# freewym/espresso

Measured on AMD Instinct MI355X. Metric: audio-hours/sec training (LibriSpeech Conformer-12 + CTC), higher is better.
Workload: dtype bf16; 1 GPU; LibriSpeech 960h Conformer-12 + CTC update step, <=26000 frames & <=24 utts per GPU, V=5004, on-GPU fbank+CMVN+SpecAugment, dropout 0.1, clip 2.0, Adam; parallelism=dp1

## Files before the change

### espresso_amd/csrc/optim.hip

```cpp
#include "common.h"
#include "espresso_amd.h"

namespace {

__global__ __launch_bounds__(256) void sumsq_kernel(const float* __restrict__ g, long n, float* __restrict__ out) {
  __shared__ float sm[16];
  float s = 0.f;
  const long stride = (long)gridDim.x * blockDim.x * 4;
  for (long i = ((long)blockIdx.x * blockDim.x + threadIdx.x) * 4; i < n; i += stride) {
    if (i + 4 <= n) {
      const float4 v = *reinterpret_cast<const float4*>(g + i);
      s += v.x * v.x + v.y * v.y + v.z * v.z + v.w * v.w;
    } else {
      for (long j = i; j < n; ++j) s += g[j] * g[j];
    }
  }
  s = block_sum(s, sm);
  if (threadIdx.x == 0) atomicAdd(out, s);
}

__global__ void clip_coef_kernel(const float* __restrict__ sumsq, float pre_scale, const float* __restrict__ denom,
                                 float max_norm, float* __restrict__ coef) {
  if (denom) pre_scale = pre_scale / denom[0];
  const float norm = sqrtf(sumsq[0]) * pre_scale;
  float c = 1.f;
  if (max_norm > 0.f) c = fminf(1.f, max_norm / (norm + 1e-6f));
  if (!(fabsf(norm) < INFINITY)) c = norm;
  coef[0] = pre_scale * c;
  coef[1] = norm;
}

__global__ __launch_bounds__(256) void adam_kernel(float* __restrict__ p, float* __restrict__ g, float* __restrict__ m,
                                                   float* __restrict__ v, bf16_t* __restrict__ p_bf16, long n,
                                                   const float* __restrict__ coef, float lr, float beta1, float beta2,
                                                   float eps, float weight_decay, float step_size, int zero_grad) {
  const float gs = coef ? coef[0] : 1.f;
  const bool skip = !(gs == gs) || fabsf(gs) == INFINITY;
  const long stride = (long)gridDim.x * blockDim.x * 4;
  for (long i = ((long)blockIdx.x * blockDim.x + threadIdx.x) * 4; i < n; i += stride) {
    const int cnt = (int)((n - i) < 4 ? (n - i) : 4);
    float pv[4], gv[4], mv[4], vv[4];
    if (cnt == 4) {
      const f32x4_t a = __builtin_nontemporal_load(reinterpret_cast<const f32x4_t*>(p + i));
      const f32x4_t b = __builtin_nontemporal_load(reinterpret_cast<const f32x4_t*>(g + i));
      const f32x4_t c = __builtin_nontemporal_load(reinterpret_cast<const f32x4_t*>(m + i));
      const f32x4_t d = __builtin_nontemporal_load(reinterpret_cast<const f32x4_t*>(v + i));
      pv[0] = a.x; pv[1] = a.y; pv[2] = a.z; pv[3] = a.w;
// ... 24 lines not shown
      if (zero_grad) __builtin_nontemporal_store((f32x4_t){0.f, 0.f, 0.f, 0.f}, reinterpret_cast<f32x4_t*>(g + i));
      if (p_bf16) *reinterpret_cast<uint2*>(p_bf16 + i) = make_uint2(pack_bf2(pv[0], pv[1]), pack_bf2(pv[2], pv[3]));
    } else {
      for (int e = 0; e < cnt; ++e) {
        p[i + e] = pv[e]; m[i + e] = mv[e]; v[i + e] = vv[e];
        if (zero_grad) g[i + e] = 0.f;
        if (p_bf16) p_bf16[i + e] = f2bf(pv[e]);
      }
    }
  }
}

}

extern "C" int ea_grad_sumsq(const float* g, long n, float* out , hipStream_t stream) {
  if (n <= 0) return 0;
  long blocks = (n + 1023) / 1024;
  if (blocks > 2048) blocks = 2048;
  hipLaunchKernelGGL(sumsq_kernel, dim3((unsigned)blocks), dim3(256), 0, stream, g, n, out);
  return EA_CHECK_LAUNCH();
}
extern "C" int ea_clip_coef(const float* sumsq, float pre_scale, const float* denom_dev, float max_norm,
                            float* coef , hipStream_t stream) {
  hipLaunchKernelGGL(clip_coef_kernel, dim3(1), dim3(1), 0, stream, sumsq, pre_scale, denom_dev, max_norm, coef);
  return EA_CHECK_LAUNCH();
}
extern "C" int ea_adam_step(float* p, float* g, float* m, float* v, void* p_bf16, long n, const float* coef,
                            float lr, float beta1, float beta2, float eps, float weight_decay, int step,
                            int zero_grad, hipStream_t stream) {
  if (n <= 0) return 0;
  const double bc1 = 1.0 - pow((double)beta1, (double)step);
  const double bc2 = 1.0 - pow((double)beta2, (double)step);
  const float step_size = (float)((double)lr * sqrt(bc2) / bc1);
  long blocks = (n + 1023) / 1024;
  if (blocks > 4096) blocks = 4096;
  hipLaunchKernelGGL(adam_kernel, dim3((unsigned)blocks), dim3(256), 0, stream, p, g, m, v, (bf16_t*)p_bf16, n, coef, lr,
                     beta1, beta2, eps, weight_decay, step_size, zero_grad);
  return EA_CHECK_LAUNCH();
}
```

### espresso_amd/functional.py

```python
import collections

import ctypes
import os

import torch

from . import kernels as K

_seed_state = {"base": 0x5EED, "counter": 0}


def set_dropout_seed(seed: int):
    _seed_state["base"] = int(seed) & 0xFFFFFFFF
    _seed_state["counter"] = 0


_seed_trace = None


class trace_dropout_seeds:

    def __enter__(self):
        global _seed_trace
        self.prev, self.entries = _seed_trace, []
# ... 644 lines not shown


_CONV1_FUSED_BWD = True


def set_conv1_fused_backward(on: bool) -> bool:
    global _CONV1_FUSED_BWD
    old, _CONV1_FUSED_BWD = _CONV1_FUSED_BWD, bool(on)
    return old


def set_conv_implicit_gemm(on: bool):
    global _CONV_IGEMM
    _CONV_IGEMM = bool(on)


def _conv_igemm_ok(cin, cout, sy, sx):
    return _CONV_IGEMM and cin in (64, 128) and cout in (64, 128) and sy in (1, 2) and sx in (1, 2)


class _ConvSubsample(torch.autograd.Function):

    @staticmethod
    def forward(ctx, X, row_zero, strides, bufs, p_drop, training, bn_eps, bn_momentum, *params):
        B, T, F = X.shape
        L = len(params) // 4
        saved = []
        cfgs = []
        A = None
        Tc, Fc, Cc = T, F, 1
        for i in range(L):
            w, b, g, beta = params[4 * i: 4 * i + 4]
            rm, rv = bufs[2 * i], bufs[2 * i + 1]
            sy, sx = strides[i]
            Co = w.shape[0]
            To, Fo = (Tc - 1) // sy + 1, (Fc - 1) // sx + 1
            stats = _pool_zeros((2 * Co,), torch.float64, X.device) if training else None
            if i == 0:
                assert w.shape[1] == 1 and tuple(w.shape[2:]) == (3, 3)
                Zi = K.conv1_fwd(X, w.detach().reshape(Co, 9).contiguous(), b, B, Tc, Fc, Co, sy, sx, stats)
                col, w16 = None, None
            elif _conv_igemm_ok(Cc, Co, sy, sx):
                w16 = K.cast_f32_to_bf16(w.detach().permute(0, 2, 3, 1).reshape(Co, 9 * Cc).contiguous())
                Zi = K.conv3x3_fwd(A, w16, b, B, Tc, Fc, Cc, Co, sy, sx, stats=stats)
                col = A
            else:
                col = K.im2col3x3(A, B, Tc, Fc, Cc, sy, sx)
                w16 = K.cast_f32_to_bf16(w.detach().permute(0, 2, 3, 1).reshape(Co, 9 * Cc).contiguous())
                Zi = _new((B * To * Fo, Co), torch.bfloat16, X)
                K.gemm(col, w16, Zi, B * To * Fo, Co, 9 * Cc, lda=9 * Cc, ldb=9 * Cc, ldc=Co, bias=b)
                if training:
                    K.colstats(Zi, stats)
            n = B * To * Fo
            mr = K.bn_finalize(stats, Co, n, bn_eps, bn_momentum, rm, rv) if training else K.bn_from_running(rm, rv, bn_eps)
            A = K.bn_act_fwd(Zi, mr, g, beta, "relu")
            saved += [Zi, mr, col, w16, g, beta]
            cfgs.append((Tc, Fc, Cc, To, Fo, Co, sy, sx))
            Tc, Fc, Cc = To, Fo, Co
        out = A.view(B * Tc, Fc * Cc)
        seed = _next_seed("subsample.out", p_drop) if (training and p_drop > 0) else 0
        if seed:
            out = K.scale_dropout(out, a=1.0, drop_p=p_drop, drop_seed=seed)
        if row_zero is not None:
            K.zero_rows(out, row_zero)
        ctx.save_for_backward(X, row_zero, *[t for t in saved if t is not None])
        ctx.layout = [[t is not None for t in saved[6 * i: 6 * i + 6]] for i in range(L)]
        ctx.cfg = (B, cfgs, p_drop, seed, training, [tuple(p.shape) for p in params[0::4]])
        ctx.igemm = [i > 0 and _conv_igemm_ok(cfgs[i][2], cfgs[i][5], cfgs[i][6], cfgs[i][7]) for i in range(L)]
        ctx.weights = [params[4 * i] for i in range(L)]
        ctx.params = list(params)
        return out

    @staticmethod
    def backward(ctx, dout):
        X, row_zero, *flat = ctx.saved_tensors
        B, cfgs, p_drop, seed, training, wshapes = ctx.cfg
        L = len(cfgs)
        it = iter(flat)
# ... 59 lines not shown
                    grads[4 * i] = dWp.view(Co, 3, 3, Cc).permute(0, 3, 1, 2)
                if not training:
                    db = g.detach() * mr[1] * dbeta
                elif _grad_sink(pb, Co) is not None:
                    db = None
                wd16 = K.cast_f32_to_bf16(ctx.weights[i].detach().permute(1, 2, 3, 0).reshape(Cc, 9 * Co).contiguous())
                dA = K.conv3x3_dgrad(dZ, wd16, B, Tc, Fc, Cc, Co, sy, sx)
            else:
                dWp = torch.empty((Co, 9 * Cc), dtype=torch.float32, device=X.device)
                side.wait_stream(cur)
                with torch.cuda.stream(side):
                    _wgrad(dZ, col, n, Co, 9 * Cc, out=dWp)
                    K.colsum(dZ, db, n, Co, Co)
                grads[4 * i] = dWp.view(Co, 3, 3, Cc).permute(0, 3, 1, 2)
                dcol = _new((n, 9 * Cc), torch.bfloat16, X)
                K.gemm(dZ, w16, dcol, n, 9 * Cc, Co, lda=Co, ldb=9 * Cc, ldc=9 * Cc, b_kstrided=True)
                dA = K.col2im3x3(dcol, B, Tc, Fc, Cc, sy, sx)
            grads[4 * i + 1] = db
            if sg is None:
                grads[4 * i + 2] = dg
                grads[4 * i + 3] = dbeta
        cur.wait_stream(side)
        del keep
        return (None,) * 8 + tuple(grads)


def conv_subsample(X, row_zero, strides, params, bufs, p_drop=0.0, training=True, bn_eps=1e-5, bn_momentum=0.1):
    return _ConvSubsample.apply(X, row_zero, tuple(strides), list(bufs), p_drop, training, bn_eps, bn_momentum, *params)


_grad_ready_callback = None


def set_grad_ready_callback(fn):
    global _grad_ready_callback
    _grad_ready_callback = fn


def _ptr(t):
    return None if t is None else t.data_ptr()


class _LayerBinding:

    def __init__(self, m, kind="conformer"):
        import ctypes

        from ._lib import EaConformerLayer

        self.keep = []
        self.kind = kind
# ... 1277 lines not shown
```

### espresso_amd/kernels.py

```python
import ctypes
from typing import Optional

import torch

from . import _lib
from ._lib import EaGemmParams, check

ACT_NONE, ACT_RELU, ACT_SILU = 0, 1, 2
_ACT = {None: 0, "none": 0, "relu": 1, "silu": 2, "swish": 2}


def _stream():
    return ctypes.c_void_p(torch._C._cuda_getCurrentRawStream(torch._C._cuda_getDevice()))


def _p(t: Optional[torch.Tensor]):
    if t is None:
        return None
    if not t.is_cuda:
        raise RuntimeError("espresso_amd kernels need device tensors (no CPU path)")
    return ctypes.c_void_p(t.data_ptr())


def drop_params(p: float):
# ... 457 lines not shown
        "ea_specaugment",
    )
    return feat


def grad_sumsq(g, out):
    check(_lib.lib().ea_grad_sumsq(_p(g), g.numel(), _p(out), _stream()), "ea_grad_sumsq")
    return out


def clip_coef(sumsq, pre_scale, max_norm, coef, denom_dev=None):
    check(_lib.lib().ea_clip_coef(_p(sumsq), pre_scale, _p(denom_dev), max_norm, _p(coef), _stream()), "ea_clip_coef")
    return coef


def adam_step(p, g, m, v, p_bf16, coef, lr, beta1, beta2, eps, weight_decay, step, zero_grad=True):
    check(
        _lib.lib().ea_adam_step(_p(p), _p(g), _p(m), _p(v), _p(p_bf16), p.numel(), _p(coef), lr, beta1, beta2, eps,
                                weight_decay, step, int(zero_grad), _stream()),
        "ea_adam_step",
    )


def ctc_greedy_decode(x, in_len, B, T, V, blank, pad, ld=None, want_align=True):
    dev = x.device
    ld = x.stride(0) if ld is None else ld
    best = torch.empty(B * T, dtype=torch.int32, device=dev)
    bestv = torch.empty(B * T, dtype=torch.float32, device=dev)
    tokens = torch.empty(B, T, dtype=torch.int32, device=dev)
    align = torch.zeros(B, T, dtype=torch.int32, device=dev) if want_align else None
    out_len = torch.empty(B, dtype=torch.int32, device=dev)
    score = torch.empty(B, dtype=torch.float32, device=dev)
    check(
        _lib.lib().ea_ctc_greedy_decode(_p(x), ld, int(x.dtype == torch.bfloat16), _p(in_len), _p(best), _p(bestv), _p(tokens),
                                        _p(align), _p(out_len), _p(score), B, T, V, blank, pad, _stream()),
        "ea_ctc_greedy_decode",
    )
    return tokens, out_len, score, align


def _finish_outputs(n, nbest, max_u, device):
    return (torch.empty(n, nbest, max_u, dtype=torch.int32, device=device), torch.empty(n, nbest, dtype=torch.int32, device=device),
            torch.empty(n, nbest, dtype=torch.float32, device=device), torch.empty(n, dtype=torch.int32, device=device))


def _partial_outputs(n, max_u, device):
# ... 1135 lines not shown
```

### espresso_amd/models/transformer/speech_transformer_encoder_model.py

```python
import os

import torch
import torch.nn as nn

from ... import functional as F
from ... import kernels as K
from ...modules.conformer_layer import ConformerWithRelativePositionalEmbeddingEncoderLayer
from ...modules.params import LayerNormParams, LinearParams
from ...modules.learned_relative_positional_embedding import LearnedRelativePositionalEmbedding
from ...modules.sinusoidal_relative_positional_embedding import SinusoidalRelativePositionalEmbedding
from ...modules.speech_convolutions import ConvBNReLU
from ...modules.transformer_layer import TransformerWithRelativePositionalEmbeddingEncoderLayer
from ...registry import register_model, register_model_architecture
from ...tools import utils as speech_utils
from .speech_transformer_config import DEFAULT_MAX_SOURCE_POSITIONS, SpeechTransformerConfig

_LOGITS_F32 = os.environ.get("EA_LOGITS_F32", "0") == "1"


class AbsolutePositionTable(nn.Module):

    def __init__(self, num_embeddings, dim):
        super().__init__()
        self.weight = nn.Parameter(torch.empty(num_embeddings, dim))
# ... 29 lines not shown
                rels = [LearnedRelativePositionalEmbedding(dim, max_size=size)] * nl
            else:
                rels = [LearnedRelativePositionalEmbedding(dim, max_size=size) for _ in range(nl)]
        else:
            rels = [SinusoidalRelativePositionalEmbedding(d)] * nl
        self.rel_pos_embed = [rels[0]]
        if getattr(cfg.encoder, "depthwise_conv_causal", False) and cfg.encoder.layer_type != "conformer":
            raise ValueError(f"encoder.depthwise_conv_causal needs encoder.layer_type: conformer (got {cfg.encoder.layer_type}: "
                             "only the conformer layer has a depthwise convolution)")
        if cfg.encoder.layer_type == "conformer":
            layer_cls = ConformerWithRelativePositionalEmbeddingEncoderLayer
        elif cfg.encoder.layer_type == "transformer":
            layer_cls = TransformerWithRelativePositionalEmbeddingEncoderLayer
        else:
            raise NotImplementedError(cfg.encoder.layer_type)
        self.layers = nn.ModuleList([layer_cls(cfg, positional_embedding=rels[i]) for i in range(nl)])
        self.num_layers = len(self.layers)
        if cfg.encoder.normalize_before and cfg.encoder.layer_type != "conformer":
            self.layer_norm = LayerNormParams(d)
        else:
            self.layer_norm = None
        self.transformer_context = speech_utils.eval_str_nested_list_or_tuple(cfg.encoder.transformer_context, type=int)
        self.num_updates = 0

    def set_num_updates(self, num_updates):
        self.num_updates = num_updates

    def output_lengths(self, in_lengths):
        return in_lengths if self.pre_encoder is None else self.pre_encoder.output_lengths(in_lengths)

    def get_attn_mask(self, max_len, device, in_lengths=None):
        if self.cfg.encoder.chunk_size > 0:
            from ...data.data_utils import numpy_seed

            with numpy_seed(self.num_updates):
                vis = speech_utils.chunk_streaming_mask(in_lengths, self.cfg.encoder.chunk_size,
                                                        left_window=self.cfg.encoder.chunk_left_window,
                                                        right_window=self.cfg.encoder.chunk_right_window,
                                                        always_partial_in_last=not self.training)
            return torch.zeros(max_len, max_len, device=device).masked_fill(~vis.to(device), -1e8).contiguous()
        tc = self.transformer_context
        if tc is None or (tc[0] is None and tc[1] is None):
            return None
        ones = torch.ones(max_len, max_len, dtype=torch.bool, device=device)
        if tc[0] is None:
            m = ones.triu(tc[1] + 1)
        elif tc[1] is None:
            m = ones.tril(-tc[0] - 1)
        else:
# ... 53 lines not shown
        x, x_lengths, padding_mask, row_zero = self.pre_encoder(src_tokens, src_lengths, p_drop=p if self.fc0 is not None else 0.0)
        Tp = padding_mask.shape[1]
        if self.fc0 is not None:
            x = F.linear(x, self._fc0_weight(), self.fc0.bias)
        if self.abs_positions or self.embed_scale != 1.0:
            x = self._add_positions(x, padding_mask)
        if self.layernorm_embedding is not None:
            x = F.layer_norm(x, self.layernorm_embedding.weight, self.layernorm_embedding.bias, row_zero=row_zero, drop_p=p)
        else:
            if p > 0:
                x = F.dropout(x, p)
            if row_zero is not None:
                x = F.zero_rows(x, row_zero)
        key_len = x_lengths.to(torch.int32).contiguous()
        attn_mask = self.get_attn_mask(Tp, x.device, in_lengths=x_lengths)
        states = [x] if return_all_hiddens else []
        ld = float(getattr(cfg.encoder, "layerdrop", 0.0) or 0.0)
        keep = torch.empty(len(self.layers)).uniform_() > ld if (tr and ld > 0) else None
        wt_event = None
        if tr and torch.is_grad_enabled() and x.is_cuda:
            native = [l for i, l in enumerate(self.layers) if (keep is None or bool(keep[i])) and _native_conformer(l)]
            if native:
                wt_event = F.refresh_layer_transposes(native, B, Tp)
        kept = [l for i, l in enumerate(self.layers) if keep is None or bool(keep[i])]
        if (not return_all_hiddens and x.is_cuda and all(_native_conformer(l) for l in kept) and F.conformer_stack_supported(kept, x)):
            l0 = kept[0]
            c0 = l0.cfg
            x = F.conformer_stack_native(x, kept, key_len, attn_mask, l0.positional_embedding[0].table(Tp, x.device), B, Tp,
                                         c0.dropout if tr else 0.0, c0.activation_dropout if tr else 0.0,
                                         c0.attention_dropout if tr else 0.0, tr)
            if tr:
                for l in kept:
                    if not getattr(l, "_counters_managed", False):
                        l.conv_module.batch_norm.num_batches_tracked += 1
            kept = []
        for i, layer in enumerate(kept):        kept = [l for i, l in enumerate(self.layers) if keep is None or bool(keep[i])]
        for i, layer in enumerate(kept):
            nxt = kept[i + 1] if i + 1 < len(kept) else None
            if nxt is not None and not return_all_hiddens and x.is_cuda and _native_conformer(layer) and _native_conformer(nxt):
                x = layer(x, B, Tp, key_len=key_len, attn_mask=attn_mask, chain_next=nxt)
            else:
                x = layer(x, B, Tp, key_len=key_len, attn_mask=attn_mask)
            if return_all_hiddens:
                states.append(x)
        if wt_event is not None:
            torch.cuda.current_stream(x.device).wait_event(wt_event)
# ... 69 lines not shown
        ev = speech_utils.eval_str_nested_list_or_tuple
        out_channels = ev(cfg.encoder.conv_channels, type=int)
        kernel_sizes = ev(cfg.encoder.conv_kernel_sizes, type=int)
        strides = ev(cfg.encoder.conv_strides, type=int)
        assert task.feat_dim % task.feat_in_channels == 0
        conv_layers = ConvBNReLU(out_channels, kernel_sizes, strides, in_channels=task.feat_in_channels) if out_channels is not None else None
        in_size = task.feat_dim // task.feat_in_channels
        if conv_layers is not None:
            in_size = conv_layers.output_feat_dim(in_size)
        else:
            in_size = task.feat_dim
        vocab = len(task.target_dictionary) if task.target_dictionary is not None else None
        encoder = cls.build_encoder(cfg, pre_encoder=conv_layers, input_size=in_size, vocab_size=vocab)
        return cls(cfg, encoder)

    @classmethod
    def build_encoder(cls, cfg, pre_encoder=None, input_size=83, vocab_size=None):
        return SpeechTransformerEncoderForPrediction(cfg, pre_encoder=pre_encoder, input_size=input_size, vocab_size=vocab_size)

    def set_num_updates(self, num_updates):
        self.num_updates = num_updates
        self.encoder.set_num_updates(num_updates)

    def forward(self, src_tokens, src_lengths, **kwargs):
        return self.encoder(src_tokens, src_lengths, **kwargs)

    def output_lengths(self, in_lengths):
        return self.encoder.output_lengths(in_lengths)

    def max_positions(self):
        return self.encoder.max_positions()

    def get_normalized_probs(self, net_output, log_probs, sample=None):
        lg = net_output.get("_logits_bt")
        if lg:
            logits = lg[0]
            B, Tp = net_output["encoder_padding_mask"][0].shape
        else:
            e = net_output["encoder_out"][0]
            Tp, B, V = e.shape
            logits = e.transpose(0, 1).reshape(B * Tp, V)
        M, V = logits.shape
        lp = K.log_softmax(logits.detach(), M, V, logits.stride(0))
        if not log_probs:
            lp = lp.exp_()
        return lp.view(B, Tp, V).transpose(0, 1)
# ... 32 lines not shown
```

### espresso_amd/modules/speech_convolutions.py

```python
import torch
import torch.nn as nn

from .. import functional as F
from .params import BatchNormParams, ConvParams


class ConvBNReLU(nn.Module):
    def __init__(self, out_channels, kernel_sizes, strides, in_channels=1, apply_batchnorm=True):
        super().__init__()
        assert apply_batchnorm, "the MI355X path implements the recipes' BatchNorm variant"
        assert in_channels == 1, "fbank input has one channel (task.feat_in_channels == 1)"
        self.out_channels, self.kernel_sizes, self.strides, self.in_channels = out_channels, kernel_sizes, strides, in_channels
        self.convolutions = nn.ModuleList()
        self.batchnorms = nn.ModuleList()
        for i, co in enumerate(out_channels):
            ks = kernel_sizes[i]
            ks = tuple(ks) if isinstance(ks, (list, tuple)) else (ks, ks)
            assert ks == (3, 3), "3x3 kernels (all recipes)"
            self.convolutions.append(ConvParams(in_channels if i == 0 else out_channels[i - 1], co, ks))
            self.batchnorms.append(BatchNormParams(co))

    def _stride2(self, s):
        if isinstance(s, (list, tuple)):
            return (s[0], s[1] if len(s) > 1 else s[0])
# ... 16 lines not shown

    def output_feat_dim(self, feat_dim):
        f = feat_dim
        for stride in self.strides:
            s = self._stride2(stride)[1]
            f = (f + s - 1) // s
        return f * self.out_channels[-1]

    def forward(self, src, src_lengths, p_drop=0.0):
        B, T, _ = src.shape
        x_lengths = self.output_lengths(src_lengths)
        Tp = (T + 0)
        for stride in self.strides:
            s = self._stride2(stride)[0]
            Tp = (Tp + s - 1) // s
        padding_mask = torch.arange(Tp, device=src.device).unsqueeze(0) >= x_lengths.unsqueeze(1)
        row_zero = padding_mask.reshape(-1).to(torch.uint8).contiguous()
        params, bufs = [], []
        for conv, bn in zip(self.convolutions, self.batchnorms):
            params += [conv.weight, conv.bias, bn.weight, bn.bias]
            bufs += [bn.running_mean, bn.running_var]
        x = F.conv_subsample(src.contiguous().float(), row_zero, [self._stride2(s) for s in self.strides], params, bufs,
                             p_drop=p_drop, training=self.training, bn_eps=self.batchnorms[0].eps,
                             bn_momentum=self.batchnorms[0].momentum)
        if self.training and not getattr(self, "_counters_managed", False):
            for bn in self.batchnorms:
                bn.num_batches_tracked += 1
        return x, x_lengths, padding_mask, row_zero
```

### espresso_amd/optim/adam.py

```python
import torch

from .. import kernels as K
from ..registry import register_optimizer
from .flat import FlatParams


@register_optimizer("adam")
class FlatAdam:
    def __init__(self, flat: FlatParams, lr=1e-3, betas=(0.9, 0.999), eps=1e-8, weight_decay=0.0):
        self.flat = flat
        self.lr, self.betas, self.eps, self.weight_decay = lr, betas, eps, weight_decay
        dev = flat.p32.device
        self.exp_avg = torch.zeros_like(flat.p32)
        self.exp_avg_sq = torch.zeros_like(flat.p32)
        self.step_count = 0
        self._sumsq = torch.zeros(1, dtype=torch.float32, device=dev)
        self._coef = torch.zeros(2, dtype=torch.float32, device=dev)

    def set_lr(self, lr):
        self.lr = lr

    def get_lr(self):
        return self.lr

    def clip_and_step(self, pre_scale=1.0, max_norm=0.0, denom_dev=None):
        f = self.flat
        self._sumsq.zero_()
        K.grad_sumsq(f.g32, self._sumsq)
        K.clip_coef(self._sumsq, pre_scale, max_norm, self._coef, denom_dev)
        self.step_count += 1
        K.adam_step(f.p32, f.g32, self.exp_avg, self.exp_avg_sq, f.p16, self._coef, self.lr, self.betas[0], self.betas[1],
                    self.eps, self.weight_decay, self.step_count, zero_grad=True)
        return self._coef

    def state_dict(self):
        return {"step": self.step_count, "exp_avg": self.exp_avg, "exp_avg_sq": self.exp_avg_sq, "lr": self.lr}

    def load_state_dict(self, sd):
        self.step_count = sd["step"]
        self.exp_avg.copy_(sd["exp_avg"])
        self.exp_avg_sq.copy_(sd["exp_avg_sq"])
        self.lr = sd.get("lr", self.lr)
```

### espresso_amd/optim/flat.py

```python
from typing import Dict, List

import torch

from .. import kernels as K

_ALIGN = 64


class FlatParams:
    def __init__(self, module: torch.nn.Module, device=None):
        from ..modules.conformer_layer import MultiheadAttentionParams

        params: List[torch.nn.Parameter] = []
        seen = set()
        fused = []
        for m in module.modules():
            if isinstance(m, MultiheadAttentionParams) and m.q_proj.weight.shape == m.k_proj.weight.shape == m.v_proj.weight.shape:
                grp = [m.q_proj.weight, m.k_proj.weight, m.v_proj.weight]
                if all(id(p) not in seen for p in grp) and grp[0].numel() % _ALIGN == 0:
                    fused.append(grp)
                    for p in grp:
                        seen.add(id(p))
                        params.append(p)
                bgrp = [m.q_proj.bias, m.k_proj.bias, m.v_proj.bias]
                if all(b is not None and id(b) not in seen for b in bgrp) and bgrp[0].numel() % _ALIGN == 0:
                    for p in bgrp:
                        seen.add(id(p))
                        params.append(p)
        for p in module.parameters():
# ... 2 lines not shown
                params.append(p)
        self.params = params
        device = device or params[0].device
        self.offsets: Dict[int, int] = {}
        off = 0
        for p in params:
            self.offsets[id(p)] = off
            off += (p.numel() + _ALIGN - 1) // _ALIGN * _ALIGN
        self.numel = off
        self.p32 = torch.zeros(off, dtype=torch.float32, device=device)
        self.g32 = torch.zeros(off, dtype=torch.float32, device=device)
        self.p16 = torch.zeros(off, dtype=torch.bfloat16, device=device)
        with torch.no_grad():
            for p in params:
                o, n = self.offsets[id(p)], p.numel()
                self.p32[o:o + n].copy_(p.data.reshape(-1))
                p.data = self.p32[o:o + n].view(p.shape)
                p.grad = self.g32[o:o + n].view(p.shape)
                p._ea_bf16 = self.p16[o:o + n].view(p.shape)
        for grp in fused:
            o = self.offsets[id(grp[0])]
            n = grp[0].numel()
            grp[0]._ea_fused_qkv = self.p16[o:o + 3 * n].view(3 * grp[0].shape[0], grp[0].shape[1])
        self.sync_bf16()

    def sync_bf16(self):
        if self.p32.is_cuda:
            K.cast_f32_to_bf16(self.p32, self.p16)

    def rebind_grads(self):
        for p in self.params:
            o, n = self.offsets[id(p)], p.numel()
            p.grad = self.g32[o:o + n].view(p.shape)

    def zero_grad(self):
        self.g32.zero_()
        self.rebind_grads()

    def slices_in_backward_order(self, bucket_elems: int, last_elems: int = 0):
        out = []
        end = self.numel
        tail = min(max(0, int(last_elems)), self.numel) if last_elems and self.numel > bucket_elems else 0
        while end > tail:
            start = max(tail, end - bucket_elems)
            out.append((start, end))
            end = start
        if tail:
# ... 3 lines not shown
```

### espresso_amd/trainer.py

```python
import contextlib

import torch
import torch.distributed as dist

from . import functional as F
from .distributed.overlapped_ddp import OverlappedDistributedDataParallel
from .optim.adam import FlatAdam
from .optim.flat import FlatParams
from .optim.noam_lr_scheduler import NoamSchedule


def grad_norms_inconsistent(norms: torch.Tensor) -> torch.Tensor:
    g0 = norms[0]
    close = ((norms - g0).abs().max() / (g0 + 1e-6)) < 1e-6
    all_bad = (~torch.isfinite(norms)).all()
    return (~(close | all_bad)).to(torch.float32).reshape(1)


class Trainer:
    def __init__(self, task, model, criterion, device, clip_norm=2.0, lr=5.0, warmup_steps=25000, adam_betas=(0.9, 0.98),
                 adam_eps=1e-8, weight_decay=0.0, final_lr=1e-6, seed=1, bucket_mb=64.0, lr_scheduler=None):
        self.task, self.criterion, self.device = task, criterion, device
        self.model = model.to(device)
        self.flat = FlatParams(self.model, device)
        self.optimizer = FlatAdam(self.flat, lr=lr, betas=adam_betas, eps=adam_eps, weight_decay=weight_decay)
        if lr_scheduler is None:
            self.lr_scheduler = NoamSchedule(self.optimizer, lr=lr, warmup_steps=warmup_steps,
                                             model_size=model.cfg.encoder.embed_dim, final_lr=final_lr)
        else:
            from . import registry
            from .optim import lr_schedulers

            name, kw = lr_scheduler
            self.lr_scheduler = registry.LR_SCHEDULER_REGISTRY[name](self.optimizer, lr=lr, **kw)
        self.cfg = None
        self._optim_history = []
        self.world_size = dist.get_world_size() if dist.is_initialized() else 1
        self.ddp = OverlappedDistributedDataParallel(self.model, self.flat, bucket_mb=bucket_mb)
        self.clip_norm = clip_norm
        self.seed = seed
        self.num_updates = 0
        self._stats = torch.zeros(4 + (self.world_size if self.world_size > 1 else 0), dtype=torch.float32, device=device)
        self._gnorm_mismatch = torch.zeros(1, dtype=torch.float32, device=device)
        self.last_coef = None
        self.ooms = 0
        self._train_mode_checked = False

    def train_step(self, samples):
        F.set_dropout_seed(self.seed + self.num_updates)
        if not self.model.training or not self._train_mode_checked:
            self.model.train()
            self._train_mode_checked = True
        self._stats.zero_()
        F.begin_step(self._stats.device)
        for i, sample in enumerate(samples):
            last = i == len(samples) - 1
            ctx = contextlib.nullcontext() if last else self.ddp.no_sync()
            dummy = bool(sample.get("_dummy", False))
            try:
                with ctx:
                    sample = self.task.prepare_sample(sample, train=True)
                    loss, sample_size, log = self.criterion(self.ddp, sample)
                    if dummy:
                        loss = loss * 0.0
                    with F.accumulating_backward():
                        loss.backward()
            except RuntimeError as e:
                if "out of memory" not in str(e).lower():
                    raise
                self._recover_from_oom(e)
                return None
            if dummy:
                continue
            self._stats[0:1].add_(float(sample_size))
            self._stats[1:2].add_(loss.detach().reshape(1))
            self._stats[2:3].add_(float(log["ntokens"]))
            self._stats[3:4].add_(float(log["nsentences"]))
        if self.ddp.active:
            if self.world_size > 1 and self.last_coef is not None:
                self._stats[4 + dist.get_rank():5 + dist.get_rank()].copy_(self.last_coef[1:2])
            dist.all_reduce(self._stats)
            if self.world_size > 1 and self.last_coef is not None:
                self._gnorm_mismatch += grad_norms_inconsistent(self._stats[4:])
        self.ddp.all_reduce_grads()
        F.end_step()
        self.last_coef = self.optimizer.clip_and_step(pre_scale=1.0, max_norm=self.clip_norm, denom_dev=self._stats[0:1])
        self.num_updates += 1
        if hasattr(self.model, "set_num_updates"):
            self.model.set_num_updates(self.num_updates)
        self.lr_scheduler.step_update(self.num_updates)
        return self._stats[:4]

    def _recover_from_oom(self, exc):
        import sys

        self.ooms += 1
        print(f"| WARNING: ran out of memory in the forward/backward pass of update {self.num_updates + 1} ({exc}); "
              f"{'skipping the update' if self.world_size == 1 else 'cannot skip on one rank of ' + str(self.world_size)}", file=sys.stderr)
        if self.world_size > 1:
            raise RuntimeError("out of memory on one data-parallel rank: gradient buckets of this update may already be in flight, "
                               "the update cannot be skipped consistently (lower max_tokens / batch_size)") from exc
        F.end_step()
        for m in self.model.modules():
            b = getattr(m, "_ea_binding", None)
            if b is not None:
                b.saved_busy = False
            m.__dict__.pop("_ea_chain_in", None)
            m.__dict__.pop("_ea_wt_fresh", None)
        self.flat.zero_grad()
        self._stats.zero_()
        if self._stats.is_cuda:
            torch.cuda.synchronize(self._stats.device)
            torch.cuda.empty_cache()

    def check_grad_norm_consistency(self):
        bad = float(self._gnorm_mismatch)
        self._gnorm_mismatch.zero_()
        if bad > 0:
            raise FloatingPointError(
                f"Fatal error: gradients are inconsistent between workers ({int(bad)} update(s) since the last check). "
                "Try --ddp-backend=legacy_ddp. Or are you mixing up different generation of GPUs in training?")

    def reserve(self, samples):
        bn = {n: b.clone() for n, b in self.model.named_buffers()}
        self.model.train()
        with self.ddp.no_sync():
            for sample in samples:
                sample = self.task.prepare_sample(sample, train=True)
                loss, _, _ = self.criterion(self.ddp, sample)
                with F.accumulating_backward():
                    loss.backward()
        self.flat.zero_grad()
        with torch.no_grad():
            for n, b in self.model.named_buffers():
                b.copy_(bn[n])
        if torch.cuda.is_available():
            torch.cuda.synchronize()

    def valid_step(self, sample):
        return self.task.valid_step(sample, self.model, self.criterion)


    @classmethod
    def from_cfg(cls, cfg, task, model, criterion, device):
        from .config import as_list, literal

        opt, optim = cfg["optimization"], cfg["optimizer"]
        if optim.get("_name", "adam") != "adam":
            raise NotImplementedError(f"optimizer {optim.get('_name')!r} (every ASR recipe of the reference uses adam)")
        sched = dict(cfg["lr_scheduler"])
        name = sched.pop("_name")
        sched.pop("lr", None)
        if name in ("reduce_lr_on_plateau_v2", "reduce_lr_on_plateau"):
            sched.setdefault("maximize_best_checkpoint_metric", cfg["checkpoint"]["maximize_best_checkpoint_metric"])
        if name == "tri_stage":
            sched.setdefault("max_update", opt["max_update"])
            if sched.get("phase_ratio") is not None:
                sched["phase_ratio"] = literal(sched["phase_ratio"])
        t = cls(task, model, criterion, device, clip_norm=float(opt["clip_norm"]), lr=float(as_list(opt["lr"])[0]),
                adam_betas=tuple(literal(optim["adam_betas"])), adam_eps=float(optim["adam_eps"]),
                weight_decay=float(optim["weight_decay"]), seed=int(cfg["common"]["seed"]), lr_scheduler=(name, sched))
        t.cfg = cfg
        return t

    def get_lr(self):
        return self.optimizer.get_lr()

    def lr_step_begin_epoch(self, epoch):
        if hasattr(self.lr_scheduler, "step_begin_epoch"):
            self.lr_scheduler.step_begin_epoch(epoch)
        return self.get_lr()

    def lr_step(self, epoch, val_loss=None):
        if hasattr(self.lr_scheduler, "step"):
            self.lr_scheduler.step(epoch, val_loss)
        return self.get_lr()

    def _optimizer_state(self):
        f, o = self.flat, self.optimizer
        state, ids = {}, []
        for i, p in enumerate(q for q in self.model.parameters() if q.requires_grad):
            off, n = f.offsets[id(p)], p.numel()
            state[i] = {"step": o.step_count, "exp_avg": o.exp_avg[off:off + n].view(p.shape).clone().cpu(),
                        "exp_avg_sq": o.exp_avg_sq[off:off + n].view(p.shape).clone().cpu()}
            ids.append(i)
        group = {"lr": o.lr, "betas": tuple(o.betas), "eps": o.eps, "weight_decay": o.weight_decay, "amsgrad": False, "params": ids}
        return {"state": state, "param_groups": [group]}

    def _load_optimizer_state(self, sd):
        f, o = self.flat, self.optimizer
        params = [q for q in self.model.parameters() if q.requires_grad]
        if len(sd["state"]) not in (0, len(params)):
            raise ValueError(f"optimizer state holds {len(sd['state'])} parameters, the model has {len(params)}")
        for i, p in enumerate(params):
            st = sd["state"].get(i)
            if st is None:
                continue
            off, n = f.offsets[id(p)], p.numel()
            o.exp_avg[off:off + n].copy_(st["exp_avg"].reshape(-1))
            o.exp_avg_sq[off:off + n].copy_(st["exp_avg_sq"].reshape(-1))
            o.step_count = int(st["step"])
        if sd.get("param_groups"):
            o.lr = sd["param_groups"][0].get("lr", o.lr)

    def state_dict(self, extra_state=None):
        sched = self.lr_scheduler.state_dict() if hasattr(self.lr_scheduler, "state_dict") else {}
        extra = {"previous_training_time": 0.0}
        extra.update(extra_state or {})
        no_optim = bool(((self.cfg or {}).get("checkpoint") or {}).get("no_save_optimizer_state", False))
        sd = {
            "args": None,
            "cfg": self.cfg,
            "model": {k: v.detach().clone().cpu() for k, v in self.model.state_dict().items()},
            "criterion": None,
            "optimizer_history": self._optim_history + [{
                "criterion_name": type(self.criterion).__name__, "optimizer_name": type(self.optimizer).__name__,
                "lr_scheduler_state": sched, "num_updates": self.num_updates}],
            "task_state": {},
            "extra_state": extra,
        }
        if not no_optim:
            sd["last_optimizer_state"] = self._optimizer_state()
        return sd

    def save_checkpoint(self, filename, extra_state=None):
        import os

        if dist.is_initialized() and dist.get_rank() != 0:
            return
        tmp = filename + ".tmp"
        torch.save(self.state_dict(extra_state), tmp)
        os.replace(tmp, filename)

    def load_checkpoint(self, filename, reset_optimizer=False, reset_lr_scheduler=False):
        import os

        if not os.path.exists(filename):
            return None
        state = torch.load(filename, map_location="cpu", weights_only=False)
        sd = state["model"]
        if hasattr(self.model, "upgrade_state_dict_named"):
            sd = self.model.upgrade_state_dict_named(dict(sd), "")
        with torch.no_grad():
            own = self.model.state_dict()
            missing = [k for k in own if k not in sd]
            unexpected = [k for k in sd if k not in own]
            if missing or unexpected:
                raise RuntimeError(f"checkpoint does not match the model: missing {missing[:5]}, unexpected {unexpected[:5]}")
            for k, v in own.items():
                v.copy_(sd[k])
        self.flat.sync_bf16()
        hist = state.get("optimizer_history") or []
        self._optim_history = hist[:-1]
        last = hist[-1] if hist else None
        if last is not None and not reset_optimizer and state.get("last_optimizer_state") is not None:
            if last["criterion_name"] != type(self.criterion).__name__:
                raise RuntimeError("Criterion does not match; please reset the optimizer (--reset-optimizer)")
            self._load_optimizer_state(state["last_optimizer_state"])
            self.num_updates = int(last["num_updates"])
            if hasattr(self.model, "set_num_updates"):
                self.model.set_num_updates(self.num_updates)
            if not reset_lr_scheduler and hasattr(self.lr_scheduler, "load_state_dict") and last.get("lr_scheduler_state"):
                self.lr_scheduler.load_state_dict(last["lr_scheduler_state"])
            self.lr_scheduler.step_update(self.num_updates)
        return state.get("extra_state") or {}
```

### include/espresso_amd.h

```cpp
#ifndef ESPRESSO_AMD_H
#define ESPRESSO_AMD_H

#include <stdint.h>

#ifdef __cplusplus
extern "C" {
#endif

typedef struct ihipStream_t* ea_stream_t;

int ea_version(void);

enum { EA_ACT_NONE = 0, EA_ACT_RELU = 1, EA_ACT_SILU = 2 };

typedef struct EaGemmParams {
  const void* A;
  const void* B;
  void* C;
  void* C2;
  const float* bias;
  const void* resid;
  const void* aux;
  int M, N, K, batch, zdiv;
  int a_kstrided, b_kstrided, c_f32, accumulate, resid_f32, act;
// ... 347 lines not shown
                             const int* token_host, const void* keep_host, int N, int* ctx_out_host, float* rows_host, long ld);
int ea_label_smoothed_ce(const void* logits, long ld, int logits_bf16, const int* target, float* out_loss,
                         void* dlogits, long ld_out, int dlogits_bf16, long M, int V, int pad_idx, float eps,
                         float grad_scale, int smoothing, const float* prior, int tgt_len, ea_stream_t stream);

int ea_fbank_batch(const float* wav, const long* offsets, int B, const float* window, const float* twiddle,
                   const int* mel_start, const int* mel_len, const int* mel_woff, const float* mel_w,
                   const float* cmvn_mean, const float* cmvn_std, float* feat, float* utt_sum, int* out_len,
                   int Tmax, int nmel, int frame_len, int frame_shift, float preemph, float log_floor,
                   ea_stream_t stream);
int ea_fbank_batch_i16(const int16_t* wav, const long* offsets, int B, const float* window, const float* twiddle,
                   const int* mel_start, const int* mel_len, const int* mel_woff, const float* mel_w,
                   const float* cmvn_mean, const float* cmvn_std, float* feat, float* utt_sum, int* out_len,
                   int Tmax, int nmel, int frame_len, int frame_shift, float preemph, float log_floor,
                   ea_stream_t stream);
int ea_specaugment(float* feat, const int* lengths, const float* utt_sum, const int* fmask, const int* tmask,
                   int nf, int nt, int B, int Tmax, int nmel, int use_mean, float mask_value, ea_stream_t stream);

int ea_feature_stats(const float* feat, const int* lengths, double* acc, int B, int Tmax, int nmel, ea_stream_t stream);

int ea_grad_sumsq(const float* g, long n, float* out, ea_stream_t stream);
int ea_clip_coef(const float* sumsq, float pre_scale, const float* denom_dev, float max_norm, float* coef,
                 ea_stream_t stream);
int ea_adam_step(float* p, float* g, float* m, float* v, void* p_bf16, long n, const float* coef, float lr,
                 float beta1, float beta2, float eps, float weight_decay, int step, int zero_grad,
                 ea_stream_t stream);

typedef struct EaFfnParams { const float *ln_g, *ln_b; const void* w1; const float* b1; const void* w2; const float* b2; } EaFfnParams;
typedef struct EaFfnGrads { float *ln_g, *ln_b, *w1, *b1, *w2, *b2; } EaFfnGrads;
typedef struct EaAttnParams {
  const float *ln_g, *ln_b; const void* wqkv; const float* bqkv; const void* wo; const float* bo;
  const float *pos_u, *pos_v; const void* wpos;
} EaAttnParams;
typedef struct EaAttnGrads { float *ln_g, *ln_b, *wqkv, *bqkv, *wo, *bo, *pos_u, *pos_v, *wpos; } EaAttnGrads;
typedef struct EaConvParams {
  const float *ln_g, *ln_b; const void* pw1; const float* dw; const float *bn_g, *bn_b; float *bn_rm, *bn_rv; const void* pw2;
} EaConvParams;
typedef struct EaConvGrads { float *ln_g, *ln_b, *pw1, *dw, *bn_g, *bn_b, *pw2; } EaConvGrads;
typedef struct EaLayerGrads { EaFfnGrads ffn1; EaAttnGrads attn; EaConvGrads conv; EaFfnGrads ffn2; float *final_ln_g, *final_ln_b; } EaLayerGrads;
typedef struct EaConformerLayer {
  EaFfnParams ffn1; EaAttnParams attn; EaConvParams conv; EaFfnParams ffn2; const float *final_ln_g, *final_ln_b;
  EaLayerGrads grads;
  void* wt;
} EaConformerLayer;
typedef struct EaLayerShape {
  int B, T, C, H, F, KW, training; float p_drop, p_act, p_attn; uint64_t seed; int has_attn_mask;
  int scratch_clean;
  int pos_mode, act;
  int S;
// ... 189 lines not shown
```

Baseline: 5.385 audio-hours/sec.

## Defer Adam update of late parameters to overlap with next forward pass

```diff
diff --git a/espresso_amd/csrc/optim.hip b/espresso_amd/csrc/optim.hip
--- a/espresso_amd/csrc/optim.hip
+++ b/espresso_amd/csrc/optim.hip
@@ -19,10 +19,11 @@
   if (threadIdx.x == 0) atomicAdd(out, s);
 }
 
-__global__ void clip_coef_kernel(const float* __restrict__ sumsq, float pre_scale, const float* __restrict__ denom,
-                                 float max_norm, float* __restrict__ coef) {
+__global__ void clip_coef_kernel(float* __restrict__ sumsq, float pre_scale, const float* __restrict__ denom, float max_norm,
+                                 float* __restrict__ coef, int clear) {
   if (denom) pre_scale = pre_scale / denom[0];
   const float norm = sqrtf(sumsq[0]) * pre_scale;
+  if (clear) sumsq[0] = 0.f;
   float c = 1.f;
   if (max_norm > 0.f) c = fminf(1.f, max_norm / (norm + 1e-6f));
   if (!(fabsf(norm) < INFINITY)) c = norm;
@@ -93,19 +94,35 @@
 }
 extern "C" int ea_clip_coef(const float* sumsq, float pre_scale, const float* denom_dev, float max_norm,
                             float* coef , hipStream_t stream) {
-  hipLaunchKernelGGL(clip_coef_kernel, dim3(1), dim3(1), 0, stream, sumsq, pre_scale, denom_dev, max_norm, coef);
+  hipLaunchKernelGGL(clip_coef_kernel, dim3(1), dim3(1), 0, stream, const_cast<float*>(sumsq), pre_scale, denom_dev, max_norm,
+                     coef, 0);
+  return EA_CHECK_LAUNCH();
+}
+extern "C" int ea_clip_coef_clear(float* sumsq, float pre_scale, const float* denom_dev, float max_norm, float* coef ,
+                                  hipStream_t stream) {
+  hipLaunchKernelGGL(clip_coef_kernel, dim3(1), dim3(1), 0, stream, sumsq, pre_scale, denom_dev, max_norm, coef, 1);
+  return EA_CHECK_LAUNCH();
+}
+static int adam_launch(float* p, float* g, float* m, float* v, void* p_bf16, long n, const float* coef, float lr, float beta1,
+                       float beta2, float eps, float weight_decay, int step, int zero_grad, long max_blocks, hipStream_t stream) {
+  if (n <= 0) return 0;
+  const double bc1 = 1.0 - pow((double)beta1, (double)step);
+  const double bc2 = 1.0 - pow((double)beta2, (double)step);
+  const float step_size = (float)((double)lr * sqrt(bc2) / bc1);
+  long blocks = (n + 1023) / 1024;
+  if (blocks > max_blocks) blocks = max_blocks;
+  hipLaunchKernelGGL(adam_kernel, dim3((unsigned)blocks), dim3(256), 0, stream, p, g, m, v, (bf16_t*)p_bf16, n, coef, lr,
+                     beta1, beta2, eps, weight_decay, step_size, zero_grad);
   return EA_CHECK_LAUNCH();
 }
 extern "C" int ea_adam_step(float* p, float* g, float* m, float* v, void* p_bf16, long n, const float* coef,
                             float lr, float beta1, float beta2, float eps, float weight_decay, int step,
                             int zero_grad, hipStream_t stream) {
-  if (n <= 0) return 0;
-  const double bc1 = 1.0 - pow((double)beta1, (double)step);
-  const double bc2 = 1.0 - pow((double)beta2, (double)step);
-  const float step_size = (float)((double)lr * sqrt(bc2) / bc1);
-  long blocks = (n + 1023) / 1024;
-  if (blocks > 4096) blocks = 4096;
-  hipLaunchKernelGGL(adam_kernel, dim3((unsigned)blocks), dim3(256), 0, stream, p, g, m, v, (bf16_t*)p_bf16, n, coef, lr,
-                     beta1, beta2, eps, weight_decay, step_size, zero_grad);
-  return EA_CHECK_LAUNCH();
+  return adam_launch(p, g, m, v, p_bf16, n, coef, lr, beta1, beta2, eps, weight_decay, step, zero_grad, 4096, stream);
 }
+extern "C" int ea_adam_step_capped(float* p, float* g, float* m, float* v, void* p_bf16, long n, const float* coef,
+                                   float lr, float beta1, float beta2, float eps, float weight_decay, int step,
+                                   int zero_grad, int max_blocks, hipStream_t stream) {
+  if (max_blocks < 1) return n <= 0 ? 0 : -1;
+  return adam_launch(p, g, m, v, p_bf16, n, coef, lr, beta1, beta2, eps, weight_decay, step, zero_grad, max_blocks, stream);
+}
diff --git a/espresso_amd/functional.py b/espresso_amd/functional.py
--- a/espresso_amd/functional.py
+++ b/espresso_amd/functional.py
@@ -690,7 +690,7 @@
 class _ConvSubsample(torch.autograd.Function):
 
     @staticmethod
-    def forward(ctx, X, row_zero, strides, bufs, p_drop, training, bn_eps, bn_momentum, *params):
+    def forward(ctx, X, row_zero, strides, bufs, p_drop, training, bn_eps, bn_momentum, after_first_layer, *params):
         B, T, F = X.shape
         L = len(params) // 4
         saved = []
@@ -722,6 +722,8 @@
             n = B * To * Fo
             mr = K.bn_finalize(stats, Co, n, bn_eps, bn_momentum, rm, rv) if training else K.bn_from_running(rm, rv, bn_eps)
             A = K.bn_act_fwd(Zi, mr, g, beta, "relu")
+            if i == 0 and after_first_layer is not None:
+                after_first_layer()
             saved += [Zi, mr, col, w16, g, beta]
             cfgs.append((Tc, Fc, Cc, To, Fo, Co, sy, sx))
             Tc, Fc, Cc = To, Fo, Co
@@ -827,11 +829,13 @@
                 grads[4 * i + 3] = dbeta
         cur.wait_stream(side)
         del keep
-        return (None,) * 8 + tuple(grads)
-
-
-def conv_subsample(X, row_zero, strides, params, bufs, p_drop=0.0, training=True, bn_eps=1e-5, bn_momentum=0.1):
-    return _ConvSubsample.apply(X, row_zero, tuple(strides), list(bufs), p_drop, training, bn_eps, bn_momentum, *params)
+        return (None,) * 9 + tuple(grads)
+
+
+def conv_subsample(X, row_zero, strides, params, bufs, p_drop=0.0, training=True, bn_eps=1e-5, bn_momentum=0.1,
+                   after_first_layer=None):
+    return _ConvSubsample.apply(X, row_zero, tuple(strides), list(bufs), p_drop, training, bn_eps, bn_momentum, after_first_layer,
+                                *params)
 
 
 _grad_ready_callback = None
diff --git a/espresso_amd/kernels.py b/espresso_amd/kernels.py
--- a/espresso_amd/kernels.py
+++ b/espresso_amd/kernels.py
@@ -503,6 +503,19 @@
     )
 
 
+def clip_coef_clear(sumsq, pre_scale, max_norm, coef, denom_dev=None):
+    check(_lib.lib().ea_clip_coef_clear(_p(sumsq), pre_scale, _p(denom_dev), max_norm, _p(coef), _stream()), "ea_clip_coef_clear")
+    return coef
+
+
+def adam_step_capped(p, g, m, v, p_bf16, coef, lr, beta1, beta2, eps, weight_decay, step, max_blocks, stream, zero_grad=True):
+    check(
+        _lib.lib().ea_adam_step_capped(_p(p), _p(g), _p(m), _p(v), _p(p_bf16), p.numel(), _p(coef), lr, beta1, beta2, eps,
+                                       weight_decay, step, int(zero_grad), int(max_blocks), ctypes.c_void_p(stream.cuda_stream)),
+        "ea_adam_step_capped",
+    )
+
+
 def ctc_greedy_decode(x, in_len, B, T, V, blank, pad, ld=None, want_align=True):
     dev = x.device
     ld = x.stride(0) if ld is None else ld
diff --git a/espresso_amd/models/transformer/speech_transformer_encoder_model.py b/espresso_amd/models/transformer/speech_transformer_encoder_model.py
--- a/espresso_amd/models/transformer/speech_transformer_encoder_model.py
+++ b/espresso_amd/models/transformer/speech_transformer_encoder_model.py
@@ -75,9 +75,19 @@
             self.layer_norm = None
         self.transformer_context = speech_utils.eval_str_nested_list_or_tuple(cfg.encoder.transformer_context, type=int)
         self.num_updates = 0
+        self.pending_update = None
+        if pre_encoder is not None:
+            pre_encoder.after_first_layer = self.start_pending_update
 
     def set_num_updates(self, num_updates):
         self.num_updates = num_updates
+
+    def start_pending_update(self):
+        if self.pending_update is not None:
+            self.pending_update.start()
+
+    def early_modules(self):
+        return [self.pre_encoder, self.fc0, self.embed_positions, self.layernorm_embedding]
 
     def output_lengths(self, in_lengths):
         return in_lengths if self.pre_encoder is None else self.pre_encoder.output_lengths(in_lengths)
@@ -177,6 +187,9 @@
             native = [l for i, l in enumerate(self.layers) if (keep is None or bool(keep[i])) and _native_conformer(l)]
             if native:
                 wt_event = F.refresh_layer_transposes(native, B, Tp)
+        if self.pending_update is not None:
+            self.pending_update.wait(torch.cuda.current_stream(x.device))
+            self.pending_update = None
         kept = [l for i, l in enumerate(self.layers) if keep is None or bool(keep[i])]
         if (not return_all_hiddens and x.is_cuda and all(_native_conformer(l) for l in kept) and F.conformer_stack_supported(kept, x)):
             l0 = kept[0]
@@ -292,6 +305,19 @@
         self.num_updates = num_updates
         self.encoder.set_num_updates(num_updates)
 
+    def early_update_modules(self):
+        return self.encoder.early_modules()
+
+    def defer_update(self, pending):
+        self.encoder.pending_update = pending
+
+    def state_dict(self, *args, **kwargs):
+        if self.encoder.pending_update is not None:
+            dev = next(self.parameters()).device
+            self.encoder.pending_update.wait(torch.cuda.current_stream(dev))
+            self.encoder.pending_update = None
+        return super().state_dict(*args, **kwargs)
+
     def forward(self, src_tokens, src_lengths, **kwargs):
         return self.encoder(src_tokens, src_lengths, **kwargs)
 
diff --git a/espresso_amd/modules/speech_convolutions.py b/espresso_amd/modules/speech_convolutions.py
--- a/espresso_amd/modules/speech_convolutions.py
+++ b/espresso_amd/modules/speech_convolutions.py
@@ -62,7 +62,7 @@
             bufs += [bn.running_mean, bn.running_var]
         x = F.conv_subsample(src.contiguous().float(), row_zero, [self._stride2(s) for s in self.strides], params, bufs,
                              p_drop=p_drop, training=self.training, bn_eps=self.batchnorms[0].eps,
-                             bn_momentum=self.batchnorms[0].momentum)
+                             bn_momentum=self.batchnorms[0].momentum, after_first_layer=getattr(self, "after_first_layer", None))
         if self.training and not getattr(self, "_counters_managed", False):
             for bn in self.batchnorms:
                 bn.num_batches_tracked += 1
diff --git a/espresso_amd/optim/adam.py b/espresso_amd/optim/adam.py
--- a/espresso_amd/optim/adam.py
+++ b/espresso_amd/optim/adam.py
@@ -3,6 +3,26 @@
 from .. import kernels as K
 from ..registry import register_optimizer
 from .flat import FlatParams
+
+SIDE_MAX_BLOCKS = 256
+
+
+class PendingUpdate:
+
+    def __init__(self, launch):
+        self._launch, self._event = launch, None
+
+    @property
+    def started(self):
+        return self._event is not None
+
+    def start(self):
+        if self._event is None:
+            self._event, self._launch = self._launch(), None
+        return self._event
+
+    def wait(self, stream):
+        stream.wait_event(self.start())
 
 
 @register_optimizer("adam")
@@ -33,6 +53,28 @@
                     self.eps, self.weight_decay, self.step_count, zero_grad=True)
         return self._coef
 
+    def clip_and_step_split(self, side_stream, pre_scale=1.0, max_norm=0.0, denom_dev=None, hold=False):
+        f = self.flat
+        lo, hi = f.early_range
+        K.grad_sumsq(f.g32, self._sumsq)
+        K.clip_coef_clear(self._sumsq, pre_scale, max_norm, self._coef, denom_dev)
+        self.step_count += 1
+        args = (self._coef, self.lr, self.betas[0], self.betas[1], self.eps, self.weight_decay, self.step_count)
+        cut = lambda a, b: (f.p32[a:b], f.g32[a:b], self.exp_avg[a:b], self.exp_avg_sq[a:b], f.p16[a:b])
+        K.adam_step(*cut(lo, hi), *args, zero_grad=True)
+
+        def launch():
+            side_stream.wait_stream(torch.cuda.current_stream(f.p32.device))
+            for a, b in ((0, lo), (hi, f.numel)):
+                if b > a:
+                    K.adam_step_capped(*cut(a, b), *args, SIDE_MAX_BLOCKS, side_stream, zero_grad=True)
+            return side_stream.record_event()
+
+        pending = PendingUpdate(launch)
+        if not hold:
+            pending.start()
+        return self._coef, pending
+
     def state_dict(self):
         return {"step": self.step_count, "exp_avg": self.exp_avg, "exp_avg_sq": self.exp_avg_sq, "lr": self.lr}
 
diff --git a/espresso_amd/optim/flat.py b/espresso_amd/optim/flat.py
--- a/espresso_amd/optim/flat.py
+++ b/espresso_amd/optim/flat.py
@@ -5,6 +5,7 @@
 from .. import kernels as K
 
 _ALIGN = 64
+_EARLY_MAX_SHARE = 0.25
 
 
 class FlatParams:
@@ -53,7 +54,22 @@
             o = self.offsets[id(grp[0])]
             n = grp[0].numel()
             grp[0]._ea_fused_qkv = self.p16[o:o + 3 * n].view(3 * grp[0].shape[0], grp[0].shape[1])
+        declared = getattr(module, "early_update_modules", None)
+        self.early_range = self.range_of(declared()) if callable(declared) else None
         self.sync_bf16()
+
+    def range_of(self, modules, max_share=_EARLY_MAX_SHARE):
+        inside = {id(p) for m in modules if m is not None for p in m.parameters() if id(p) in self.offsets}
+        if not inside:
+            return None
+        span = lambda p: (self.offsets[id(p)], self.offsets[id(p)] + (p.numel() + _ALIGN - 1) // _ALIGN * _ALIGN)
+        lo = min(span(p)[0] for p in self.params if id(p) in inside)
+        hi = max(span(p)[1] for p in self.params if id(p) in inside)
+        if any(id(p) not in inside and span(p)[0] < hi and span(p)[1] > lo for p in self.params):
+            return None
+        if hi - lo > max_share * self.numel:
+            return None
+        return lo, hi
 
     def sync_bf16(self):
         if self.p32.is_cuda:
diff --git a/espresso_amd/trainer.py b/espresso_amd/trainer.py
--- a/espresso_amd/trainer.py
+++ b/espresso_amd/trainer.py
@@ -19,24 +19,24 @@
 
 class Trainer:
     def __init__(self, task, model, criterion, device, clip_norm=2.0, lr=5.0, warmup_steps=25000, adam_betas=(0.9, 0.98),
-                 adam_eps=1e-8, weight_decay=0.0, final_lr=1e-6, seed=1, bucket_mb=64.0, lr_scheduler=None):
+                 adam_eps=1e-8, weight_decay=0.0, final_lr=1e-6, seed=1, bucket_mb=64.0, lr_scheduler=None, defer_update=True):
         self.task, self.criterion, self.device = task, criterion, device
         self.model = model.to(device)
-        self.flat = FlatParams(self.model, device)
-        self.optimizer = FlatAdam(self.flat, lr=lr, betas=adam_betas, eps=adam_eps, weight_decay=weight_decay)
+        self._flat = FlatParams(self.model, device)
+        self._optimizer = FlatAdam(self._flat, lr=lr, betas=adam_betas, eps=adam_eps, weight_decay=weight_decay)
         if lr_scheduler is None:
-            self.lr_scheduler = NoamSchedule(self.optimizer, lr=lr, warmup_steps=warmup_steps,
+            self.lr_scheduler = NoamSchedule(self._optimizer, lr=lr, warmup_steps=warmup_steps,
                                              model_size=model.cfg.encoder.embed_dim, final_lr=final_lr)
         else:
             from . import registry
             from .optim import lr_schedulers
 
             name, kw = lr_scheduler
-            self.lr_scheduler = registry.LR_SCHEDULER_REGISTRY[name](self.optimizer, lr=lr, **kw)
+            self.lr_scheduler = registry.LR_SCHEDULER_REGISTRY[name](self._optimizer, lr=lr, **kw)
         self.cfg = None
         self._optim_history = []
         self.world_size = dist.get_world_size() if dist.is_initialized() else 1
-        self.ddp = OverlappedDistributedDataParallel(self.model, self.flat, bucket_mb=bucket_mb)
+        self.ddp = OverlappedDistributedDataParallel(self.model, self._flat, bucket_mb=bucket_mb)
         self.clip_norm = clip_norm
         self.seed = seed
         self.num_updates = 0
@@ -45,9 +45,31 @@
         self.last_coef = None
         self.ooms = 0
         self._train_mode_checked = False
+        self._split_update = (bool(defer_update) and torch.device(device).type == "cuda" and self._flat.early_range is not None
+                              and hasattr(self.model, "defer_update"))
+        self._pending_update = None
+
+    @property
+    def flat(self):
+        self.flush_update()
+        return self._flat
+
+    @property
+    def optimizer(self):
+        self.flush_update()
+        return self._optimizer
+
+    def flush_update(self):
+        pending, self._pending_update = self._pending_update, None
+        if pending is not None:
+            pending.wait(torch.cuda.current_stream(self._flat.p32.device))
+            if hasattr(self.model, "defer_update"):
+                self.model.defer_update(None)
 
     def train_step(self, samples):
         F.set_dropout_seed(self.seed + self.num_updates)
+        if not self._split_update:
+            self.flush_update()
         if not self.model.training or not self._train_mode_checked:
             self.model.train()
             self._train_mode_checked = True
@@ -84,7 +106,12 @@
                 self._gnorm_mismatch += grad_norms_inconsistent(self._stats[4:])
         self.ddp.all_reduce_grads()
         F.end_step()
-        self.last_coef = self.optimizer.clip_and_step(pre_scale=1.0, max_norm=self.clip_norm, denom_dev=self._stats[0:1])
+        if self._split_update:
+            self.last_coef, self._pending_update = self._optimizer.clip_and_step_split(
+                F._side_stream(self._flat.p32.device), pre_scale=1.0, max_norm=self.clip_norm, denom_dev=self._stats[0:1], hold=True)
+            self.model.defer_update(self._pending_update)
+        else:
+            self.last_coef = self._optimizer.clip_and_step(pre_scale=1.0, max_norm=self.clip_norm, denom_dev=self._stats[0:1])
         self.num_updates += 1
         if hasattr(self.model, "set_num_updates"):
             self.model.set_num_updates(self.num_updates)
@@ -107,7 +134,8 @@
                 b.saved_busy = False
             m.__dict__.pop("_ea_chain_in", None)
             m.__dict__.pop("_ea_wt_fresh", None)
-        self.flat.zero_grad()
+        self.flush_update()
+        self._flat.zero_grad()
         self._stats.zero_()
         if self._stats.is_cuda:
             torch.cuda.synchronize(self._stats.device)
@@ -122,6 +150,7 @@
                 "Try --ddp-backend=legacy_ddp. Or are you mixing up different generation of GPUs in training?")
 
     def reserve(self, samples):
+        self.flush_update()
         bn = {n: b.clone() for n, b in self.model.named_buffers()}
         self.model.train()
         with self.ddp.no_sync():
@@ -130,7 +159,7 @@
                 loss, _, _ = self.criterion(self.ddp, sample)
                 with F.accumulating_backward():
                     loss.backward()
-        self.flat.zero_grad()
+        self._flat.zero_grad()
         with torch.no_grad():
             for n, b in self.model.named_buffers():
                 b.copy_(bn[n])
@@ -138,6 +167,7 @@
             torch.cuda.synchronize()
 
     def valid_step(self, sample):
+        self.flush_update()
         return self.task.valid_step(sample, self.model, self.criterion)
 
 
@@ -164,7 +194,7 @@
         return t
 
     def get_lr(self):
-        return self.optimizer.get_lr()
+        return self._optimizer.get_lr()
 
     def lr_step_begin_epoch(self, epoch):
         if hasattr(self.lr_scheduler, "step_begin_epoch"):
@@ -177,7 +207,8 @@
         return self.get_lr()
 
     def _optimizer_state(self):
-        f, o = self.flat, self.optimizer
+        self.flush_update()
+        f, o = self._flat, self._optimizer
         state, ids = {}, []
         for i, p in enumerate(q for q in self.model.parameters() if q.requires_grad):
             off, n = f.offsets[id(p)], p.numel()
@@ -188,7 +219,8 @@
         return {"state": state, "param_groups": [group]}
 
     def _load_optimizer_state(self, sd):
-        f, o = self.flat, self.optimizer
+        self.flush_update()
+        f, o = self._flat, self._optimizer
         params = [q for q in self.model.parameters() if q.requires_grad]
         if len(sd["state"]) not in (0, len(params)):
             raise ValueError(f"optimizer state holds {len(sd['state'])} parameters, the model has {len(params)}")
@@ -204,6 +236,7 @@
             o.lr = sd["param_groups"][0].get("lr", o.lr)
 
     def state_dict(self, extra_state=None):
+        self.flush_update()
         sched = self.lr_scheduler.state_dict() if hasattr(self.lr_scheduler, "state_dict") else {}
         extra = {"previous_training_time": 0.0}
         extra.update(extra_state or {})
@@ -214,7 +247,7 @@
             "model": {k: v.detach().clone().cpu() for k, v in self.model.state_dict().items()},
             "criterion": None,
             "optimizer_history": self._optim_history + [{
-                "criterion_name": type(self.criterion).__name__, "optimizer_name": type(self.optimizer).__name__,
+                "criterion_name": type(self.criterion).__name__, "optimizer_name": type(self._optimizer).__name__,
                 "lr_scheduler_state": sched, "num_updates": self.num_updates}],
             "task_state": {},
             "extra_state": extra,
@@ -226,6 +259,7 @@
     def save_checkpoint(self, filename, extra_state=None):
         import os
 
+        self.flush_update()
         if dist.is_initialized() and dist.get_rank() != 0:
             return
         tmp = filename + ".tmp"
@@ -235,6 +269,7 @@
     def load_checkpoint(self, filename, reset_optimizer=False, reset_lr_scheduler=False):
         import os
 
+        self.flush_update()
         if not os.path.exists(filename):
             return None
         state = torch.load(filename, map_location="cpu", weights_only=False)
@@ -249,7 +284,7 @@
                 raise RuntimeError(f"checkpoint does not match the model: missing {missing[:5]}, unexpected {unexpected[:5]}")
             for k, v in own.items():
                 v.copy_(sd[k])
-        self.flat.sync_bf16()
+        self._flat.sync_bf16()
         hist = state.get("optimizer_history") or []
         self._optim_history = hist[:-1]
         last = hist[-1] if hist else None
diff --git a/include/espresso_amd.h b/include/espresso_amd.h
--- a/include/espresso_amd.h
+++ b/include/espresso_amd.h
@@ -393,9 +393,14 @@
 int ea_grad_sumsq(const float* g, long n, float* out, ea_stream_t stream);
 int ea_clip_coef(const float* sumsq, float pre_scale, const float* denom_dev, float max_norm, float* coef,
                  ea_stream_t stream);
+int ea_clip_coef_clear(float* sumsq, float pre_scale, const float* denom_dev, float max_norm, float* coef,
+                       ea_stream_t stream);
 int ea_adam_step(float* p, float* g, float* m, float* v, void* p_bf16, long n, const float* coef, float lr,
                  float beta1, float beta2, float eps, float weight_decay, int step, int zero_grad,
                  ea_stream_t stream);
+int ea_adam_step_capped(float* p, float* g, float* m, float* v, void* p_bf16, long n, const float* coef, float lr,
+                        float beta1, float beta2, float eps, float weight_decay, int step, int zero_grad,
+                        int max_blocks, ea_stream_t stream);
 
 typedef struct EaFfnParams { const float *ln_g, *ln_b; const void* w1; const float* b1; const void* w2; const float* b2; } EaFfnParams;
 typedef struct EaFfnGrads { float *ln_g, *ln_b, *w1, *b1, *w2, *b2; } EaFfnGrads;
```

New measurement: 5.447 audio-hours/sec, median of 6. 1.01x the previous value.
